# plainerman/DiffDock-Pocket

Measured on AMD Instinct MI355X. Metric: ligand poses/sec (40 samples x 20 steps) on 3dpf, higher is better.
Workload: dtype f32 (fc and G products: fp16 hi/lo split of both operands on v_mfma_f32_16x16x32_f16 - the row-stationary conv kernel - and v_mfma_f32_32x32x16_f16, fp32 accumulate; G between its two kernels as fp16 hi + continuation byte = 19 significant bits; the exact fp32 MFMA form is timed in other_workloads)

## Files before the change

### diffdock_pocket_amd/_lib.py

```python
from __future__ import annotations

import ctypes as C
import os

HERE = os.path.dirname(os.path.abspath(__file__))
LIB_PATH = os.environ.get("DDP_HIP_LIB", os.path.join(HERE, "libddp_hip.so"))

DDP_MAX_TASKS, DDP_MAX_BLOCKS, DDP_MAX_SEGS, DDP_MAX_NS, DDP_EDGE_TILE = 9, 4, 3, 64, 64
F_SCALAR_S0, F_DOT, F_SCALAR_S1, F_VEC_S0, F_CROSS = range(5)
FS = 68

DDP_MAX_GEMM_BATCH = 16
DDP_EVAL_MAX_ATOMS = 1024
EXPORTS = ["ddp_conv_messages", "ddp_conv_rows", "ddp_stage_a_gh", "ddp_stage_a_gh3", "ddp_segment_reduce", "ddp_edge_featurize", "ddp_edge_featurize_jobs", "ddp_torsion_sh", "ddp_stage_a", "ddp_stage_a_h2",
           "ddp_pose_update", "ddp_sidechain_update", "ddp_sde_update", "ddp_radius_count", "ddp_radius_fill", "ddp_knn", "ddp_group_by_key", "ddp_node_linear", "ddp_scan_jobs", "ddp_mark_jobs", "ddp_rowcopy_jobs", "ddp_select_jobs",
           "ddp_gather_rows", "ddp_clean_pair_maps", "ddp_flex_mark", "ddp_fallback_rowmap", "ddp_step_prologue", "ddp_trrot_head", "ddp_tor_head", "ddp_radius_search_jobs", "ddp_group_by_key_jobs", "ddp_set_occupancy_shaping", "ddp_pose_rmsd", "ddp_pose_contacts", "ddp_traj_record", "ddp_abi_version", "ddp_last_error", "ddp_source_hash"]


class Seg(C.Structure):
    _fields_ = [("kind", C.c_int32), ("in_off", C.c_int32), ("count", C.c_int32)]


class Block(C.Structure):
    _fields_ = [("U", C.c_int32), ("n", C.c_int32), ("C", C.c_int32), ("out_off", C.c_int32), ("tile0", C.c_int32),
                ("ntiles", C.c_int32), ("nsub", C.c_int32), ("ups", C.c_int32), ("nseg", C.c_int32),
                ("seg", Seg * DDP_MAX_SEGS), ("g_slot", C.c_int32), ("g_col0", C.c_int32)]


class RoleSeg(C.Structure):
    _fields_ = [("block", C.c_int32), ("tile0", C.c_int32), ("tstride", C.c_int32), ("count", C.c_int32), ("round", C.c_int32)]


DDP_CONV32_WAVES, DDP_MAX_ROLE_SEGS = 4, 2


class ConvShape(C.Structure):
    _fields_ = [("f_in", C.c_int32), ("hid", C.c_int32), ("kp1", C.c_int32), ("hp", C.c_int32), ("hs", C.c_int32),
                ("nct1", C.c_int32), ("d_out", C.c_int32), ("nblocks", C.c_int32), ("fbuf_floats", C.c_int32),
                ("g_cols", C.c_int32 * 2), ("blk", Block * DDP_MAX_BLOCKS), ("nrounds", C.c_int32),
                ("nrole", C.c_int32 * DDP_CONV32_WAVES), ("role", (RoleSeg * DDP_MAX_ROLE_SEGS) * DDP_CONV32_WAVES)]


class ConvTask(C.Structure):
    _fields_ = [("x_src", C.c_void_p), ("ldx_src", C.c_int32), ("n_edges", C.c_int32), ("src", C.c_void_p),
                ("eid", C.c_void_p), ("sh", C.c_void_p), ("seg_ptr", C.c_void_p * DDP_MAX_SEGS),
                ("seg_idx", C.c_void_p * DDP_MAX_SEGS), ("seg_ld", C.c_int32 * DDP_MAX_SEGS),
                ("seg_n", C.c_int32 * DDP_MAX_SEGS), ("w1p", C.c_void_p), ("b1p", C.c_void_p), ("w2p", C.c_void_p),
# ... 93 lines not shown


def g_ld(hid: int, gcols: int) -> int:
    return (((hid + 3) // 4 * 4 + 1) * gcols + 31) // 32 * 32


class DdpError(RuntimeError):
    pass


_lib = None


def load():
    global _lib
    if _lib is not None:
        return _lib
    if not os.path.exists(LIB_PATH):
        raise DdpError(f"{LIB_PATH} not found: build it with `python -m diffdock_pocket_amd.build` "
                       f"(hipcc --offload-arch=gfx950); there is no fallback path")
    lib = C.CDLL(LIB_PATH)
    for name in EXPORTS:
        if not hasattr(lib, name):
            raise DdpError(f"{LIB_PATH} does not export {name}")
    lib.ddp_abi_version.restype = C.c_int
    lib.ddp_last_error.restype = C.c_char_p
    lib.ddp_conv_messages.argtypes = [C.POINTER(ConvShape), C.POINTER(ConvTask), C.c_int, C.c_void_p]
    lib.ddp_conv_messages.restype = C.c_int
    lib.ddp_conv_rows.argtypes = lib.ddp_conv_messages.argtypes
    lib.ddp_conv_rows.restype = C.c_int
    lib.ddp_segment_reduce.argtypes = [C.c_void_p, C.c_int, C.c_int, C.c_int, C.POINTER(ReduceSrc), C.c_int, C.c_int,
                                       C.c_int, C.c_int, C.c_void_p]
    lib.ddp_segment_reduce.restype = C.c_int
    lib.ddp_edge_featurize.argtypes = [C.c_void_p, C.c_void_p, C.c_void_p, C.c_void_p, C.c_int, C.c_void_p, C.c_void_p, C.c_int,
                                       C.c_float, C.c_void_p, C.c_void_p, C.c_int, C.c_void_p, C.c_int, C.c_int, C.c_void_p,
                                       C.c_void_p, C.c_void_p, C.c_int, C.c_void_p, C.c_void_p, C.c_void_p]
    lib.ddp_edge_featurize.restype = C.c_int
    lib.ddp_edge_featurize_jobs.argtypes = [C.POINTER(FeaturizeJob), C.c_int, C.c_void_p]
    lib.ddp_edge_featurize_jobs.restype = C.c_int
    lib.ddp_torsion_sh.argtypes = [C.c_void_p, C.c_void_p, C.c_void_p, C.c_int, C.c_void_p, C.c_void_p, C.c_void_p, C.c_int, C.c_int,
                                   C.c_void_p, C.c_void_p, C.c_int, C.c_void_p, C.c_void_p]
    lib.ddp_torsion_sh.restype = C.c_int
    lib.ddp_stage_a.argtypes = [C.c_void_p, C.c_int, C.c_int, C.c_void_p, C.c_void_p, C.c_int, C.POINTER(C.c_int32), C.c_int,
                                C.c_void_p, C.c_void_p, C.c_int, C.c_int, C.c_void_p, C.c_int, C.c_void_p]
    lib.ddp_stage_a.restype = C.c_int
    lib.ddp_stage_a_h2.argtypes = lib.ddp_stage_a.argtypes[:-1] + [C.c_void_p, C.c_void_p]
    lib.ddp_stage_a_h2.restype = C.c_int
    lib.ddp_stage_a_gh.argtypes = lib.ddp_stage_a_h2.argtypes[:-1] + [C.c_void_p, C.c_void_p]
    lib.ddp_stage_a_gh.restype = C.c_int
    lib.ddp_stage_a_gh3.argtypes = lib.ddp_stage_a_gh.argtypes
    lib.ddp_stage_a_gh3.restype = C.c_int
    lib.ddp_set_occupancy_shaping.argtypes = [C.c_int, C.c_int]
    lib.ddp_set_occupancy_shaping.restype = C.c_int
    lib.ddp_pose_update.argtypes = [C.c_void_p, C.c_int, C.c_int, C.c_void_p, C.c_void_p, C.c_void_p, C.c_int, C.c_void_p,
                                    C.c_void_p, C.c_void_p, C.c_void_p]
    lib.ddp_pose_update.restype = C.c_int
    lib.ddp_sidechain_update.argtypes = [C.c_void_p, C.c_int, C.c_int, C.c_void_p, C.c_int, C.c_void_p, C.c_void_p, C.c_void_p,
                                         C.c_void_p, C.c_void_p]
    lib.ddp_sidechain_update.restype = C.c_int
    lib.ddp_radius_count.argtypes = [C.c_void_p, C.c_void_p, C.c_void_p, C.c_void_p, C.c_int, C.c_float, C.c_int, C.c_int,
                                     C.c_void_p, C.c_void_p]
    lib.ddp_radius_count.restype = C.c_int
    lib.ddp_radius_fill.argtypes = [C.c_void_p, C.c_void_p, C.c_void_p, C.c_void_p, C.c_int, C.c_float, C.c_int, C.c_int,
                                    C.c_void_p, C.c_void_p, C.c_void_p, C.c_void_p]
    lib.ddp_radius_fill.restype = C.c_int
    lib.ddp_knn.argtypes = [C.c_void_p, C.c_void_p, C.c_void_p, C.c_int, C.c_int, C.c_void_p, C.c_void_p]
# ... 50 lines not shown
```

### diffdock_pocket_amd/csrc/ddp_misc.hip

```cpp
#include <hip/hip_runtime.h>
#include <stdlib.h>
#include <stdint.h>

#include "ddp_hip.h"
#include "ddp_internal.h"

typedef float f32x4 __attribute__((ext_vector_type(4)));

struct ReduceLaunch {
  ddp_reduce_src_t src[3];
  int nsrc;
};

__global__ void ddp_segment_reduce_kernel(float* __restrict__ x, int ldx, int n_nodes, int d_out, ReduceLaunch L,
                                          int accumulate, int n_rep, int rep_stride) {
  const int node = blockIdx.x;
  const int ch = threadIdx.x;
  if (ch >= d_out) return;
  float* dst = x + (size_t)node * ldx + ch;
  float total = (accumulate && n_rep <= 1) ? *dst : 0.f;
  int p0[3], p1[3];
#pragma unroll
  for (int k = 0; k < 3; ++k) {
    const bool on = k < L.nsrc;
// ... 6 lines not shown
      const ddp_reduce_src_t& s = L.src[k];
      const float* __restrict__ m = s.msg + ch;
      const int32_t* __restrict__ rm = s.rowmap;
      float sum = 0.f;
      for (int p = p0[k]; p < p1[k]; p += 8) {
        float v[8];
        int row[8];
#pragma unroll
        for (int i = 0; i < 8; ++i) {
          const int q = min(p + i, p1[k] - 1);
          row[i] = rm ? rm[q] : q;
        }
#pragma unroll
        for (int i = 0; i < 8; ++i) v[i] = m[(size_t)row[i] * d_out];
#pragma unroll
        for (int i = 0; i < 8; ++i)
          if (p + i < p1[k]) sum += v[i];
      }
      const int cnt = p1[k] - p0[k];
      const float mean = sum / (float)(cnt > 1 ? cnt : 1);
      total += mean * s.bn_scale[ch] + s.bn_shift[ch];
    }
  }
  if (n_rep <= 1) {
    *dst = total;
  } else {
    for (int g = 0; g < n_rep; ++g) {
      float* d = dst + (size_t)g * rep_stride * ldx;
      *d = *d + total;
    }
  }
}

typedef float red4 __attribute__((ext_vector_type(4)));
__global__ __launch_bounds__(256) void ddp_segment_reduce4_kernel(float* __restrict__ x, int ldx, int n_nodes, int d_out, ReduceLaunch L,
                                                                  int accumulate, int n_rep, int rep_stride) {
  const int nq = d_out >> 2;
  const long long item = (long long)blockIdx.x * 256 + threadIdx.x;
  const int node = (int)(item / nq), ch = 4 * (int)(item - (long long)node * nq);
  if (node >= n_nodes) return;
  float* dst = x + (size_t)node * ldx + ch;
  red4 total = (accumulate && n_rep <= 1) ? *reinterpret_cast<const red4*>(dst) : red4{0.f, 0.f, 0.f, 0.f};
  int p0[3], p1[3];
#pragma unroll
  for (int k = 0; k < 3; ++k) {
    const bool on = k < L.nsrc;
    p0[k] = on ? L.src[k].rowptr[node] : 0;
    p1[k] = on ? L.src[k].rowptr[node + 1] : 0;
  }
#pragma unroll
  for (int k = 0; k < 3; ++k) {
    if (k < L.nsrc && !(L.src[k].n_edges_dev && *L.src[k].n_edges_dev <= 0)) {
      const ddp_reduce_src_t& s = L.src[k];
      const float* __restrict__ m = s.msg + ch;
      const int32_t* __restrict__ rm = s.rowmap;
      red4 sum = {0.f, 0.f, 0.f, 0.f};
      for (int p = p0[k]; p < p1[k]; p += 8) {
        red4 v[8];
        int row[8];
#pragma unroll
        for (int i = 0; i < 8; ++i) {
          const int q = min(p + i, p1[k] - 1);
          row[i] = rm ? rm[q] : q;
        }
#pragma unroll
        for (int i = 0; i < 8; ++i) v[i] = *reinterpret_cast<const red4*>(m + (size_t)row[i] * d_out);
#pragma unroll
        for (int i = 0; i < 8; ++i)
          if (p + i < p1[k]) sum += v[i];
      }
      const int cnt = p1[k] - p0[k];
      const float den = (float)(cnt > 1 ? cnt : 1);
      const red4 sc = *reinterpret_cast<const red4*>(s.bn_scale + ch), sh = *reinterpret_cast<const red4*>(s.bn_shift + ch);
#pragma unroll
      for (int c = 0; c < 4; ++c) total[c] += (sum[c] / den) * sc[c] + sh[c];
    }
  }
  if (n_rep <= 1) {
    *reinterpret_cast<red4*>(dst) = total;
  } else {
    for (int g = 0; g < n_rep; ++g) {
      red4* d = reinterpret_cast<red4*>(dst + (size_t)g * rep_stride * ldx);
      *d = *d + total;
    }
  }
}

extern "C" int ddp_segment_reduce(float* x, int ldx, int n_nodes, int d_out, const ddp_reduce_src_t* srcs, int nsrc,
                                  int accumulate, int n_rep, int rep_stride, void* stream) {
  if (!x || (!srcs && nsrc > 0)) return ddp_fail(DDP_EINVAL, "ddp_segment_reduce: null argument");
  if (nsrc < 0 || nsrc > 3) return ddp_fail(DDP_ELIMIT, "ddp_segment_reduce: nsrc > 3");
  if (d_out < 1 || d_out > 1024) return ddp_fail(DDP_ELIMIT, "ddp_segment_reduce: d_out");
  if (n_nodes <= 0) return 0;
  ReduceLaunch L;
  L.nsrc = 0;
  for (int i = 0; i < nsrc; ++i)
    if (srcs[i].n_edges > 0) L.src[L.nsrc++] = srcs[i];
  if (L.nsrc == 0 && (accumulate || n_rep > 1)) return 0;
  if (n_rep > 1 && rep_stride < n_nodes) return ddp_fail(DDP_EINVAL, "ddp_segment_reduce: rep_stride < n_nodes");
  bool wide = ((d_out | ldx) & 3) == 0 && (reinterpret_cast<size_t>(x) & 15) == 0;
  for (int i = 0; i < L.nsrc; ++i)
    wide = wide && ((reinterpret_cast<size_t>(L.src[i].msg) | reinterpret_cast<size_t>(L.src[i].bn_scale) | reinterpret_cast<size_t>(L.src[i].bn_shift)) & 15) == 0;
  static const bool narrow_only = getenv("DDP_REDUCE_NARROW") != nullptr;
  if (wide && !narrow_only) {
    const long long items = (long long)n_nodes * (d_out >> 2);
    hipLaunchKernelGGL(ddp_segment_reduce4_kernel, dim3((unsigned)((items + 255) / 256)), dim3(256), 0, (hipStream_t)stream, x, ldx, n_nodes,
                       d_out, L, accumulate, n_rep, rep_stride);
  } else {
    const int threads = ((d_out + 63) / 64) * 64;
    hipLaunchKernelGGL(ddp_segment_reduce_kernel, dim3(n_nodes), dim3(threads), 0, (hipStream_t)stream, x, ldx, n_nodes,
                       d_out, L, accumulate, n_rep, rep_stride);
  }
  hipError_t err = hipGetLastError();
  if (err != hipSuccess) return ddp_fail_hip(err, "ddp_segment_reduce launch");
  return 0;
}

#define EF_NS 64
__global__ __launch_bounds__(256) void ddp_edge_featurize_kernel(
    const float* __restrict__ pos_a, const int* __restrict__ ia, const float* __restrict__ pos_b,
    const int* __restrict__ ib, int n_edges, const int* __restrict__ n_edges_dev, const float* __restrict__ offset, int k_rbf,
    float coeff, const float* __restrict__ pre, const int* __restrict__ pre_idx, int ld_pre, const float* __restrict__ pre2,
    int n_pre2, int ld_pre2, const float* __restrict__ w1d, const float* __restrict__ w2, const float* __restrict__ b2, int ns,
    float* __restrict__ out, float* __restrict__ sh) {
  if (n_edges_dev) n_edges = min(n_edges, *n_edges_dev);
  extern __shared__ __attribute__((aligned(16))) float smem[];
  float* s_w1 = smem;
  float* s_w2 = s_w1 + k_rbf * EF_NS;
  float* s_b2 = s_w2 + EF_NS * EF_NS;
  float* s_off = s_b2 + EF_NS;
  float* s_out = s_off + ((k_rbf + 3) & ~3);
  const int tid = threadIdx.x;
  for (int i = tid; i < k_rbf * EF_NS; i += 256) s_w1[i] = w1d[i];
  for (int i = tid; i < EF_NS * EF_NS; i += 256) s_w2[i] = w2[i];
  if (tid < EF_NS) s_b2[tid] = b2[tid];
  for (int i = tid; i < k_rbf; i += 256) s_off[i] = offset[i];
  __syncthreads();

  const int wave = tid >> 6, lane = tid & 63;
  float* my_out = s_out + wave * 64 * 65;
  for (int base = blockIdx.x * 256; base < n_edges; base += gridDim.x * 256) {
    const int e = base + tid;
    const bool live = e < n_edges;
    const int ec = live ? e : n_edges - 1;
    const int a = ia[ec], b = ib[ec];
    const float vx = pos_b[3 * b] - pos_a[3 * a], vy = pos_b[3 * b + 1] - pos_a[3 * a + 1],
                vz = pos_b[3 * b + 2] - pos_a[3 * a + 2];
    const float d = sqrtf(vx * vx + vy * vy + vz * vz);
// ... 300 lines not shown
```

### diffdock_pocket_amd/engine.py

```python
from __future__ import annotations

import ctypes as C
from collections.abc import Mapping
from types import SimpleNamespace
from typing import Dict, List, Optional

import math

import torch

from . import _lib as L
from . import graph as G
from . import launch as K
from . import packing as P
from . import packing as P_
from .graph import EdgeView

SRC_TYPE = {0: "l", 1: "r", 2: "a", 3: "a", 4: "l", 5: "r", 6: "r", 7: "l", 8: "a"}
RECV_TYPE = {0: "l", 1: "l", 2: "l", 3: "a", 4: "a", 5: "a", 6: "r", 7: "r", 8: "r"}
RECV_OF = {"a": (3, 4, 5), "r": (6, 7, 8)}
ORDER = {"l": [0, 2, 1], "a": [3, 4, 5], "r": [6, 8, 7]}
_DROP_SELF = 1


# ... 798 lines not shown
                    if sd_.n_edges > 0:
                        segs = [(e_base, sd_.eid, ns, ns), (x_recv, sd_.recv, ldx, ns), (xa, sd_.src, ldx, ns)]
                        tasks_g.append(K.make_task(pkg, path, xa, ldx, sd_, sh_k, segs, msg, g=[P.g_d.get((3, s_)) for s_ in (0, 1)]))
                    sv = c1.so_v
                    segs = [(e_base, sv.eid, ns, ns), (P.x_clean, sv.recv, ldx, ns), (P.x_clean, sv.src, ldx, ns)]
                    tasks_g.append(K.make_task(pkg, path, P.x_clean, ldx, sv, sh_k, segs, msg, g=[P.g_v.get((3, s_)) for s_ in (0, 1)]))
                    continue
                msg = torch.empty((csr.n_edges, spec.d_out), device=dev)
                P.msgs[k] = (msg, csr, pkc)
                if csr.n_edges == 0:
                    continue
                if prof_on:
                    nb_g += node_bytes(l, k)
                segs = [(e_base, so_k.eid, ns, ns), (x_recv, so_k.recv, ldx, ns), (x_src, so_k.src, ldx, ns)]
                tasks_g.append(K.make_task(conv.packed_g(dev), self._conv_path(conv, dev), x_src, ldx, so_k, sh_k, segs, msg,
                                           g=[P.gmap.get((k, s_)) for s_ in (0, 1)]))
            P.tasks_g = getattr(P, "tasks_g", []) + tasks_g
            if tasks_g:
                K.launch_convs(P.spec_g, tasks_g, flops_spec=spec, node_bytes=nb_g, tag=f"layer{l}")

        def fix_rowmaps(P):
            if P.l == 0 and F.flex0 is not None:
                for k, rm in F.flex0.rowmaps.items():
                    if k in P.msgs:
                        P.msgs[k] = (P.msgs[k][0], c[k], P.msgs[k][2], rm)

        def means(P, types):
            spec, shared = P.spec, P.shared
            for rt in types:
                if not P.active[rt]:
                    continue
                x, n = nodes[rt]
                own = [P.msgs[k] for k in ORDER[rt] if k not in shared]
                if own:
                    K.launch_reduce(x, ldx, n, spec.d_out, own, accumulate=True)
                com = [P.msgs[k] for k in ORDER[rt] if k in shared]
                if com:
                    n0 = shared[[k for k in ORDER[rt] if k in shared][0]][0]
                    K.launch_reduce(x, ldx, n0, spec.d_out, com, accumulate=True, n_rep=B, rep_stride=n0)

        if pipelined:
            P = plan(0)
            direct_tasks(P)
            if P.tasks:
                side.run(1, lambda P=P: launch_direct(P))
            stage_a(P, "lar")
            def atom_g_bytes(Pn):
                tot = 0
                for (st_, _gid), (_x, rows_, convs_) in (Pn.groups.items() if m.rows_all_or_none(dev) else ()):
                    if st_ != "a":
                        continue
                    for _k, conv_ in convs_:
                        tot += rows_[3] * 4 * sum(ld_ for ld_ in (conv_.packed_g(dev).gh_ld or []) if ld_ is not None)
                return tot
            for l in range(L_):
                nxt = plan(l + 1) if l + 1 < L_ else None
                launch_factorised(P)
                join_lists()
                fix_rowmaps(P)
                side.join(only=1)
                side.join(only=0)
                ev_r, ev_l, ev_sr, ev_sl = (torch.cuda.Event() for _ in range(4))

                def rec_chain(P=P, nxt=nxt, ev_r=ev_r, ev_sr=ev_sr):
                    means(P, "r")
                    ev_r.record()
                    if nxt is not None:
                        stage_a(nxt, "r")
                        ev_sr.record()

                def lig_chain(P=P, nxt=nxt, ev_l=ev_l, ev_sl=ev_sl):
                    means(P, "l")
# ... 184 lines not shown
```

### diffdock_pocket_amd/launch.py

```python
from __future__ import annotations

import ctypes as C
import os
from dataclasses import dataclass
from typing import Dict, List, NamedTuple, Optional, Sequence

import torch
from torch import nn

from . import _lib as L
from . import packing as P
from .graph import EdgeView


def require_hip(t: torch.Tensor):
    if not t.is_cuda:
        raise L.DdpError("the MI355X score model runs on a HIP device only (no CPU/eager fallback); "
                         "move the batch to cuda:<n>")
    L.load()


def stream():
    return C.c_void_p(torch._C._cuda_getCurrentRawStream(torch._C._cuda_getDevice()))

# ... 204 lines not shown
    t.gh_fmt, t.rows_form, t.rows_bias_k, t.rows_nts = path.gh_fmt, path.rows_form, path.rows_bias_k, path.rows_nts
    t.rows_seg0, t.rows_seg1 = path.rows_seg
    t._path = path
    t.pos = _p(view.pos)
    t.n_edges_dev = _p(view.cnt)
    t._count = (view.n_edges, view.cnt)
    return t


def launch_convs(spec: P.ConvSpec, tasks: List[L.ConvTask], flops_spec: Optional[P.ConvSpec] = None, node_bytes: float = 0.0, tag=None):
    lib = L.load()
    if not tasks:
        return
    path = tasks[0]._path
    if any((t._path.rows, t._path.rows_form) != (path.rows, path.rows_form) for t in tasks):
        raise L.DdpError("launch_convs: the tasks of one launch run through different conv kernels")
    arr = (L.ConvTask * len(tasks))(*tasks)
    shape = spec.ctypes_shape()
    prof = _PROFILER
    if prof is not None:
        e0, e1 = torch.cuda.Event(enable_timing=True), torch.cuda.Event(enable_timing=True)
        e0.record()
    if path.rows:
        L.check(lib.ddp_conv_rows(C.byref(shape), arr, len(tasks), stream()), "ddp_conv_rows")
    else:
        L.check(lib.ddp_conv_messages(C.byref(shape), arr, len(tasks), stream()), "ddp_conv_messages")
    if prof is not None:
        e1.record()
        h2 = P.h2_steps(spec) > 0 and all(t._path.h2 for t in tasks)
        prof.record_conv(e0, e1, spec, flops_spec, [t._count for t in tasks], node_bytes, tag, h2,
                         rows=(2 if path.rows_form == 1 else 1) if path.rows else 0)


def launch_reduce(x, ldx, n_nodes, d_out, sources, accumulate=True, n_rep=1, rep_stride=0):
    lib = L.load()
    arr = (L.ReduceSrc * max(len(sources), 1))()
    for i, src_ in enumerate(sources):
        msg, view, pk = src_[:3]
        arr[i].msg, arr[i].rowptr = msg.data_ptr(), view.rowptr.data_ptr()
        arr[i].bn_scale, arr[i].bn_shift, arr[i].n_edges = pk.bn_scale.data_ptr(), pk.bn_shift.data_ptr(), view.n_edges
        arr[i].rowmap = src_[3].data_ptr() if (len(src_) > 3 and src_[3] is not None) else 0
        arr[i].n_edges_dev = _p(view.cnt)
    prof = profiler(hbm=True)
    if prof is not None:
        e0, e1 = torch.cuda.Event(enable_timing=True), torch.cuda.Event(enable_timing=True)
        e0.record()
    L.check(lib.ddp_segment_reduce(ptr(x), ldx, n_nodes, d_out, arr, len(sources), 1 if accumulate else 0, n_rep, rep_stride,
                                   stream()), "ddp_segment_reduce")
    if prof is not None:
        e1.record()
        views = [s_[1] for s_ in sources]

        def nbytes(views=views, d_out=d_out, n_nodes=n_nodes, n_rep=n_rep):
            ne = sum(v.n_edges if v.cnt is None else min(v.n_edges, int(v.cnt.item())) for v in views)
            return 4.0 * d_out * (ne + 2 * n_nodes * max(n_rep, 1))
        wide = (d_out % 4 == 0 and ldx % 4 == 0 and x.data_ptr() % 16 == 0 and not os.environ.get("DDP_REDUCE_NARROW")
                and all(s_[0].data_ptr() % 16 == 0 and s_[2].bn_scale.data_ptr() % 16 == 0 and s_[2].bn_shift.data_ptr() % 16 == 0 for s_ in sources))
        prof.hbm.setdefault("ddp_segment_reduce4_kernel" if wide else "ddp_segment_reduce_kernel", []).append((e0, e1, nbytes))


class EdgeMLPPack:

    def __init__(self, seq: nn.Sequential, rbf_slice: slice, device):
        W1, b1, W2, b2 = seq[0].weight.detach(), seq[0].bias.detach(), seq[3].weight.detach(), seq[3].bias.detach()
        ns = W1.shape[0]
        k = rbf_slice.stop - rbf_slice.start
        w1d = torch.zeros(k, 64, device=device)
        w1d[:, :ns] = W1[:, rbf_slice].t()
        w2 = torch.zeros(64, 64, device=device)
        w2[:ns, :ns] = W2.t()
        b2p = torch.zeros(64, device=device)
        b2p[:ns] = b2
        self.w1d, self.w2, self.b2, self.ns, self.k = w1d.contiguous(), w2.contiguous(), b2p, ns, k
        self.W1, self.b1 = W1, b1


def edge_featurize(pack: EdgeMLPPack, dist, pos_a, ia, pos_b, ib, pre, pre_idx, pre2=None, n_edges=None, cnt=None):
    lib = L.load()
    E = int(ia.shape[0]) if n_edges is None else int(n_edges)
    dev = pos_a.device
    out = torch.empty((E, pack.ns), device=dev, dtype=torch.float32)
    sh = torch.empty((E, 4), device=dev, dtype=torch.float32)
    if E == 0:
        return out, sh
    if pre.stride(1) != 1:
        pre = pre.contiguous()
    n2 = 0 if pre2 is None else int(pre2.shape[0])
    L.check(lib.ddp_edge_featurize(ptr(pos_a), ptr(ia), ptr(pos_b), ptr(ib), E, ptr(cnt), ptr(dist.offset), pack.k,
                                   C.c_float(dist.coeff), ptr(pre), ptr(pre_idx), pre.stride(0),
                                   ptr(pre2) if n2 else None, n2, pre2.stride(0) if n2 else 0, ptr(pack.w1d),
                                   ptr(pack.w2), ptr(pack.b2), pack.ns, ptr(out), ptr(sh), stream()),
# ... 248 lines not shown
```

### include/ddp_hip.h

```cpp
#ifndef DDP_HIP_H
#define DDP_HIP_H

#include <stdint.h>

#ifdef __cplusplus
extern "C" {
#endif

#define DDP_ABI_VERSION 17
#define DDP_EINVAL (-1)
#define DDP_ELIMIT (-2)

#define DDP_MAX_TASKS 9
#define DDP_MAX_BLOCKS 4
#define DDP_MAX_SEGS 3
#define DDP_MAX_NS 64
#define DDP_EDGE_TILE 64

enum ddp_feat_kind {
  DDP_F_SCALAR_S0 = 0,
  DDP_F_DOT = 1,
  DDP_F_SCALAR_S1 = 2,
  DDP_F_VEC_S0 = 3,
  DDP_F_CROSS = 4
// ... 66 lines not shown
  const void* w2h;
  int32_t* h2_range_flag;
  const void* wsh;
  const float* bsp;
  const void* gh[2];
  int32_t gh_fmt;
  int32_t rows_form;
  int32_t rows_bias_k;
  int32_t rows_seg0, rows_seg1, rows_nts;
} ddp_conv_task_t;
#define DDP_ROWS_SX 16
#define DDP_ROWS_SW 256
#define DDP_ROWS_SH 16
#define DDP_ROWS_SG 32
#define DDP_ROWS_KPERM(ks, hh, i) (32 * ((ks) >> 1) + ((8 * ((ks) & 1) + (i)) & 3) + 8 * ((8 * ((ks) & 1) + (i)) >> 2) + 4 * (hh))
#define DDP_ROWS16_POS(j) (16 * (((j) & 7) >> 2) + 4 * ((j) >> 3) + ((j) & 3))
#define DDP_GH3_LD(hid, gcp) ((((((hid) + 7) / 8) * (gcp) + ((gcp) + 5) / 6 + 15) / 16) * 96)
#define DDP_GH_LD(hid, gcp) ((((((hid) + 7) / 8) * 8 + 1) * (gcp) + 31) / 32 * 32)
int ddp_conv_messages(const ddp_conv_shape_t* shape, const ddp_conv_task_t* tasks, int ntasks, void* stream);

int ddp_conv_rows(const ddp_conv_shape_t* shape, const ddp_conv_task_t* tasks, int ntasks, void* stream);

typedef struct {
  const float* msg;
  const int32_t* rowptr;
  const float* bn_scale;
  const float* bn_shift;
  int32_t n_edges;
  const int32_t* rowmap;
  const int32_t* n_edges_dev;
} ddp_reduce_src_t;
int ddp_segment_reduce(float* x, int ldx, int n_nodes, int d_out, const ddp_reduce_src_t* srcs, int nsrc,
                       int accumulate, int n_rep, int rep_stride, void* stream);

int ddp_edge_featurize(const float* pos_a, const int32_t* ia, const float* pos_b, const int32_t* ib, int n_edges,
                       const int32_t* n_edges_dev, const float* offset, int k_rbf, float coeff, const float* pre,
                       const int32_t* pre_idx, int ld_pre, const float* pre2, int n_pre2, int ld_pre2, const float* w1d,
                       const float* w2, const float* b2, int ns, float* out, float* sh, void* stream);

#define DDP_MAX_FEATURIZE_JOBS 8
typedef struct {
  const float* pos_a;
  const int32_t* ia;
  const float* pos_b;
  const int32_t* ib;
  int32_t n_edges;
  const int32_t* n_edges_dev;
  const float* offset;
  int32_t k_rbf;
  float coeff;
  const float* pre;
  const int32_t* pre_idx;
  int32_t ld_pre;
  const float* pre2;
  int32_t n_pre2, ld_pre2;
  const float* w1d;
  const float* w2;
  const float* b2;
  int32_t ns;
  float* out;
  float* sh;
} ddp_featurize_job_t;
int ddp_edge_featurize_jobs(const ddp_featurize_job_t* jobs, int njobs, void* stream);

int ddp_torsion_sh(const float* sh_edge, const float* bond_vec, const int32_t* bond_of_edge, int n_edges,
                   const int32_t* n_edges_dev, float* out, const float* x, int ldx, int ns, const int32_t* b0,
// ... 255 lines not shown
```

Baseline: 173.3.

## Fuse own and shared segment reductions into one software-pipelined persistent kernel

```diff
diff --git a/diffdock_pocket_amd/_lib.py b/diffdock_pocket_amd/_lib.py
--- a/diffdock_pocket_amd/_lib.py
+++ b/diffdock_pocket_amd/_lib.py
@@ -12,7 +12,7 @@
 
 DDP_MAX_GEMM_BATCH = 16
 DDP_EVAL_MAX_ATOMS = 1024
-EXPORTS = ["ddp_conv_messages", "ddp_conv_rows", "ddp_stage_a_gh", "ddp_stage_a_gh3", "ddp_segment_reduce", "ddp_edge_featurize", "ddp_edge_featurize_jobs", "ddp_torsion_sh", "ddp_stage_a", "ddp_stage_a_h2",
+EXPORTS = ["ddp_conv_messages", "ddp_conv_rows", "ddp_stage_a_gh", "ddp_stage_a_gh3", "ddp_segment_reduce", "ddp_segment_reduce_fused", "ddp_edge_featurize", "ddp_edge_featurize_jobs", "ddp_torsion_sh", "ddp_stage_a", "ddp_stage_a_h2",
            "ddp_pose_update", "ddp_sidechain_update", "ddp_sde_update", "ddp_radius_count", "ddp_radius_fill", "ddp_knn", "ddp_group_by_key", "ddp_node_linear", "ddp_scan_jobs", "ddp_mark_jobs", "ddp_rowcopy_jobs", "ddp_select_jobs",
            "ddp_gather_rows", "ddp_clean_pair_maps", "ddp_flex_mark", "ddp_fallback_rowmap", "ddp_step_prologue", "ddp_trrot_head", "ddp_tor_head", "ddp_radius_search_jobs", "ddp_group_by_key_jobs", "ddp_set_occupancy_shaping", "ddp_pose_rmsd", "ddp_pose_contacts", "ddp_traj_record", "ddp_abi_version", "ddp_last_error", "ddp_source_hash"]
 
@@ -172,6 +172,9 @@
     lib.ddp_segment_reduce.argtypes = [C.c_void_p, C.c_int, C.c_int, C.c_int, C.POINTER(ReduceSrc), C.c_int, C.c_int,
                                        C.c_int, C.c_int, C.c_void_p]
     lib.ddp_segment_reduce.restype = C.c_int
+    lib.ddp_segment_reduce_fused.argtypes = [C.c_void_p, C.c_int, C.c_int, C.c_int, C.POINTER(ReduceSrc), C.c_int, C.POINTER(ReduceSrc), C.c_int,
+                                             C.c_int, C.c_int, C.c_int, C.c_void_p]
+    lib.ddp_segment_reduce_fused.restype = C.c_int
     lib.ddp_edge_featurize.argtypes = [C.c_void_p, C.c_void_p, C.c_void_p, C.c_void_p, C.c_int, C.c_void_p, C.c_void_p, C.c_int,
                                        C.c_float, C.c_void_p, C.c_void_p, C.c_int, C.c_void_p, C.c_int, C.c_int, C.c_void_p,
                                        C.c_void_p, C.c_void_p, C.c_int, C.c_void_p, C.c_void_p, C.c_void_p]
diff --git a/diffdock_pocket_amd/csrc/ddp_misc.hip b/diffdock_pocket_amd/csrc/ddp_misc.hip
--- a/diffdock_pocket_amd/csrc/ddp_misc.hip
+++ b/diffdock_pocket_amd/csrc/ddp_misc.hip
@@ -62,58 +62,265 @@
   }
 }
 
-typedef float red4 __attribute__((ext_vector_type(4)));
-__global__ __launch_bounds__(256) void ddp_segment_reduce4_kernel(float* __restrict__ x, int ldx, int n_nodes, int d_out, ReduceLaunch L,
-                                                                  int accumulate, int n_rep, int rep_stride) {
-  const int nq = d_out >> 2;
-  const long long item = (long long)blockIdx.x * 256 + threadIdx.x;
-  const int node = (int)(item / nq), ch = 4 * (int)(item - (long long)node * nq);
-  if (node >= n_nodes) return;
-  float* dst = x + (size_t)node * ldx + ch;
-  red4 total = (accumulate && n_rep <= 1) ? *reinterpret_cast<const red4*>(dst) : red4{0.f, 0.f, 0.f, 0.f};
+#define RP_ROWS 4
+struct PipeSrc {
+  const float* msg;
+  const int32_t* rowptr;
+  const float* bn_scale;
+  const float* bn_shift;
+  const int32_t* rowmap;
+  const int32_t* n_edges_dev;
+  int com;
+};
+struct PipeJob {
+  float* x;
+  int ldx, d_out;
+  int n_rows;
+  int n_own;
+  int accumulate;
+  int n0, n_rep, rep_stride;
+  int nsrc;
+  int lpn_log2, chunks;
+  PipeSrc src[3];
+};
+
+template <int V>
+__device__ __forceinline__ void rp_load(const float* p, float (&o)[V]) {
+  if constexpr (V == 1) {
+    o[0] = *p;
+  } else {
+    typedef float vec_t __attribute__((ext_vector_type(V)));
+    const vec_t t = *reinterpret_cast<const vec_t*>(p);
+#pragma unroll
+    for (int c = 0; c < V; ++c) o[c] = t[c];
+  }
+}
+template <int V>
+__device__ __forceinline__ void rp_store(float* p, const float (&o)[V]) {
+  if constexpr (V == 1) {
+    *p = o[0];
+  } else {
+    typedef float vec_t __attribute__((ext_vector_type(V)));
+    vec_t t;
+#pragma unroll
+    for (int c = 0; c < V; ++c) t[c] = o[c];
+    *reinterpret_cast<vec_t*>(p) = t;
+  }
+}
+
+struct PipePtrs {
   int p0[3], p1[3];
-#pragma unroll
-  for (int k = 0; k < 3; ++k) {
-    const bool on = k < L.nsrc;
-    p0[k] = on ? L.src[k].rowptr[node] : 0;
-    p1[k] = on ? L.src[k].rowptr[node + 1] : 0;
-  }
-#pragma unroll
-  for (int k = 0; k < 3; ++k) {
-    if (k < L.nsrc && !(L.src[k].n_edges_dev && *L.src[k].n_edges_dev <= 0)) {
-      const ddp_reduce_src_t& s = L.src[k];
-      const float* __restrict__ m = s.msg + ch;
-      const int32_t* __restrict__ rm = s.rowmap;
-      red4 sum = {0.f, 0.f, 0.f, 0.f};
-      for (int p = p0[k]; p < p1[k]; p += 8) {
-        red4 v[8];
-        int row[8];
-#pragma unroll
-        for (int i = 0; i < 8; ++i) {
-          const int q = min(p + i, p1[k] - 1);
-          row[i] = rm ? rm[q] : q;
+  int r, j, ch;
+};
+
+template <int V>
+__global__ __launch_bounds__(256) void ddp_segment_reduce_pipe_kernel(const PipeJob J) {
+  const int lpn = 1 << J.lpn_log2, lig = (int)threadIdx.x & (lpn - 1);
+  const int slot = (int)(((long long)blockIdx.x * 256 + threadIdx.x) >> J.lpn_log2);
+  const int nslots = (int)(((long long)gridDim.x * 256) >> J.lpn_log2);
+  const int n_items = J.n_rows * J.chunks;
+  const int d_out = J.d_out;
+  bool live[3];
+#pragma unroll
+  for (int k = 0; k < 3; ++k)
+    live[k] = k < J.nsrc && !(J.src[k].n_edges_dev && *J.src[k].n_edges_dev <= 0);
+
+  auto fetch_ptrs = [&](int it, PipePtrs& P) {
+#pragma unroll
+    for (int k = 0; k < 3; ++k) P.p0[k] = P.p1[k] = -1;
+    P.r = P.j = P.ch = -1;
+    if (it < n_items) {
+      const int r = it / J.chunks, chunk = it - r * J.chunks;
+      const int ch = ((chunk << J.lpn_log2) + lig) * V;
+      if (ch < d_out) {
+        P.r = r;
+        P.ch = ch;
+        if (J.n_rep >= 1) {
+          const int g = r / J.rep_stride, jj = r - g * J.rep_stride;
+          if (g < J.n_rep && jj < J.n0) P.j = jj;
         }
 #pragma unroll
-        for (int i = 0; i < 8; ++i) v[i] = *reinterpret_cast<const red4*>(m + (size_t)row[i] * d_out);
-#pragma unroll
-        for (int i = 0; i < 8; ++i)
-          if (p + i < p1[k]) sum += v[i];
-      }
-      const int cnt = p1[k] - p0[k];
-      const float den = (float)(cnt > 1 ? cnt : 1);
-      const red4 sc = *reinterpret_cast<const red4*>(s.bn_scale + ch), sh = *reinterpret_cast<const red4*>(s.bn_shift + ch);
-#pragma unroll
-      for (int c = 0; c < 4; ++c) total[c] += (sum[c] / den) * sc[c] + sh[c];
-    }
-  }
-  if (n_rep <= 1) {
-    *reinterpret_cast<red4*>(dst) = total;
-  } else {
-    for (int g = 0; g < n_rep; ++g) {
-      red4* d = reinterpret_cast<red4*>(dst + (size_t)g * rep_stride * ldx);
-      *d = *d + total;
-    }
-  }
+        for (int k = 0; k < 3; ++k)
+          if (live[k]) {
+            const int nk = J.src[k].com ? P.j : (r < J.n_own ? r : -1);
+            if (nk >= 0) {
+              P.p0[k] = J.src[k].rowptr[nk];
+              P.p1[k] = J.src[k].rowptr[nk + 1];
+            }
+          }
+      }
+    }
+  };
+  auto fetch_map = [&](const PipePtrs& P, int (&row)[3][RP_ROWS]) {
+#pragma unroll
+    for (int k = 0; k < 3; ++k) {
+      const int32_t* __restrict__ rm = k < J.nsrc ? J.src[k].rowmap : nullptr;
+#pragma unroll
+      for (int i = 0; i < RP_ROWS; ++i) {
+        const int q = P.p0[k] + i;
+        row[k][i] = (P.p0[k] >= 0 && q < P.p1[k]) ? (rm ? rm[q] : q) : -1;
+      }
+    }
+  };
+  auto fetch_rows = [&](const PipePtrs& P, const int (&row)[3][RP_ROWS], float (&v)[3][RP_ROWS][V], float (&xv)[V]) {
+#pragma unroll
+    for (int k = 0; k < 3; ++k)
+#pragma unroll
+      for (int i = 0; i < RP_ROWS; ++i)
+        if (row[k][i] >= 0) rp_load<V>(J.src[k].msg + (size_t)row[k][i] * d_out + P.ch, v[k][i]);
+    if (P.ch >= 0 && ((P.r < J.n_own && J.accumulate) || (P.r >= J.n_own && P.j >= 0)))
+      rp_load<V>(J.x + (size_t)P.r * J.ldx + P.ch, xv);
+  };
+  auto fetch_bn = [&](const PipePtrs& P, float (&sc)[3][V], float (&sh)[3][V]) {
+    if (P.ch < 0) return;
+#pragma unroll
+    for (int k = 0; k < 3; ++k)
+      if (k < J.nsrc) {
+        rp_load<V>(J.src[k].bn_scale + P.ch, sc[k]);
+        rp_load<V>(J.src[k].bn_shift + P.ch, sh[k]);
+      }
+  };
+
+  PipePtrs P, P1, P2;
+  int row[3][RP_ROWS];
+  float v[3][RP_ROWS][V], xv[V], sc[3][V], sh[3][V];
+#pragma unroll
+  for (int c = 0; c < V; ++c) xv[c] = 0.f;
+  fetch_ptrs(slot, P);
+  fetch_ptrs(slot + nslots, P1);
+  fetch_map(P, row);
+  fetch_rows(P, row, v, xv);
+  fetch_bn(P, sc, sh);
+  for (int it = slot; it < n_items; it += nslots) {
+    int row1[3][RP_ROWS];
+    fetch_map(P1, row1);
+    fetch_ptrs(it + 2 * nslots, P2);
+    if (P.ch >= 0) {
+      float total[V], ct[V];
+      const bool from_x = (P.r < J.n_own && J.accumulate) || (P.r >= J.n_own && P.j >= 0);
+#pragma unroll
+      for (int c = 0; c < V; ++c) {
+        total[c] = from_x ? xv[c] : 0.f;
+        ct[c] = 0.f;
+      }
+#pragma unroll
+      for (int k = 0; k < 3; ++k) {
+        if (P.p0[k] < 0) continue;
+        const PipeSrc& s = J.src[k];
+        float sum[V];
+#pragma unroll
+        for (int c = 0; c < V; ++c) sum[c] = 0.f;
+#pragma unroll
+        for (int i = 0; i < RP_ROWS; ++i)
+          if (P.p0[k] + i < P.p1[k]) {
+#pragma unroll
+            for (int c = 0; c < V; ++c) sum[c] += v[k][i][c];
+          }
+        const int32_t* __restrict__ rm = s.rowmap;
+        const float* __restrict__ m = s.msg + P.ch;
+        for (int p = P.p0[k] + RP_ROWS; p < P.p1[k]; p += RP_ROWS) {
+          int rw[RP_ROWS];
+          float t[RP_ROWS][V];
+#pragma unroll
+          for (int i = 0; i < RP_ROWS; ++i) rw[i] = p + i < P.p1[k] ? (rm ? rm[p + i] : p + i) : -1;
+#pragma unroll
+          for (int i = 0; i < RP_ROWS; ++i)
+            if (rw[i] >= 0) rp_load<V>(m + (size_t)rw[i] * d_out, t[i]);
+#pragma unroll
+          for (int i = 0; i < RP_ROWS; ++i)
+            if (rw[i] >= 0) {
+#pragma unroll
+              for (int c = 0; c < V; ++c) sum[c] += t[i][c];
+            }
+        }
+        const int cnt = P.p1[k] - P.p0[k];
+        const float den = (float)(cnt > 1 ? cnt : 1);
+        if (s.com == 1) {
+#pragma unroll
+          for (int c = 0; c < V; ++c) ct[c] += (sum[c] / den) * sc[k][c] + sh[k][c];
+        } else {
+#pragma unroll
+          for (int c = 0; c < V; ++c) total[c] += (sum[c] / den) * sc[k][c] + sh[k][c];
+        }
+      }
+      if (P.j >= 0 && J.n_rep > 1) {
+#pragma unroll
+        for (int c = 0; c < V; ++c) total[c] = total[c] + ct[c];
+      }
+      if (P.r < J.n_own || P.j >= 0) rp_store<V>(J.x + (size_t)P.r * J.ldx + P.ch, total);
+    }
+    P = P1;
+    P1 = P2;
+#pragma unroll
+    for (int k = 0; k < 3; ++k)
+#pragma unroll
+      for (int i = 0; i < RP_ROWS; ++i) row[k][i] = row1[k][i];
+    fetch_rows(P, row, v, xv);
+    if (J.chunks > 1) fetch_bn(P, sc, sh);
+  }
+}
+
+template <int V>
+static long long reduce_grid_cap() {
+  static long long cap = 0;
+  if (cap == 0) {
+    int dev = 0, cus = 0, per_cu = 0;
+    if (hipGetDevice(&dev) != hipSuccess || hipDeviceGetAttribute(&cus, hipDeviceAttributeMultiprocessorCount, dev) != hipSuccess || cus <= 0) cus = 256;
+    if (hipOccupancyMaxActiveBlocksPerMultiprocessor(&per_cu, ddp_segment_reduce_pipe_kernel<V>, 256, 0) != hipSuccess || per_cu < 1) per_cu = 2;
+    (void)hipGetLastError();
+    cap = (long long)cus * (per_cu < 4 ? per_cu : 4);
+  }
+  return cap;
+}
+
+static int reduce_launch(const char* who, float* x, int ldx, int d_out, int n_own, const ddp_reduce_src_t* own, int n_own_src, int accumulate,
+                         const ddp_reduce_src_t* com, int n_com_src, int n0, int n_rep, int rep_stride, void* stream) {
+  PipeJob J;
+  J.x = x; J.ldx = ldx; J.d_out = d_out; J.n_own = n_own; J.accumulate = accumulate;
+  J.nsrc = 0;
+  for (int i = 0; i < n_own_src; ++i)
+    if (own[i].n_edges > 0 && n_own > 0) {
+      const ddp_reduce_src_t& s = own[i];
+      J.src[J.nsrc++] = PipeSrc{s.msg, s.rowptr, s.bn_scale, s.bn_shift, s.rowmap, s.n_edges_dev, 0};
+    }
+  const int n_own_live = J.nsrc;
+  for (int i = 0; i < n_com_src; ++i)
+    if (com[i].n_edges > 0 && n0 > 0 && n_rep >= 1) {
+      const ddp_reduce_src_t& s = com[i];
+      J.src[J.nsrc++] = PipeSrc{s.msg, s.rowptr, s.bn_scale, s.bn_shift, s.rowmap, s.n_edges_dev, n_rep > 1 ? 1 : 2};
+    }
+  const bool has_com = J.nsrc > n_own_live;
+  if (n_own_live == 0 && accumulate) J.n_own = 0;
+  J.n0 = has_com ? n0 : 0;
+  J.n_rep = has_com ? n_rep : 0;
+  J.rep_stride = has_com ? (n_rep > 1 ? rep_stride : n0) : 1;
+  long long rows = J.n_own;
+  if (has_com && (long long)(J.n_rep - 1) * J.rep_stride + J.n0 > rows) rows = (long long)(J.n_rep - 1) * J.rep_stride + J.n0;
+  if (rows <= 0) return 0;
+  for (int k = J.nsrc; k < 3; ++k) J.src[k] = PipeSrc{nullptr, nullptr, nullptr, nullptr, nullptr, nullptr, 0};
+  for (int k = 0; k < J.nsrc; ++k)
+    if (!J.src[k].msg || !J.src[k].rowptr || !J.src[k].bn_scale || !J.src[k].bn_shift) return ddp_fail(DDP_EINVAL, "segment reduce: a source with a null array");
+  size_t al = reinterpret_cast<size_t>(x) | ((size_t)ldx * 4) | ((size_t)d_out * 4);
+  for (int k = 0; k < J.nsrc; ++k)
+    al |= reinterpret_cast<size_t>(J.src[k].msg) | reinterpret_cast<size_t>(J.src[k].bn_scale) | reinterpret_cast<size_t>(J.src[k].bn_shift);
+  const int V = (al & 15) == 0 ? 4 : (al & 7) == 0 ? 2 : 1;
+  const int nvec = d_out / V;
+  int lg = 0;
+  while ((1 << lg) < nvec && lg < 6) ++lg;
+  J.lpn_log2 = lg;
+  J.chunks = (nvec + (1 << lg) - 1) >> lg;
+  if (rows * J.chunks > 0x7fe00000LL) return ddp_fail(DDP_ELIMIT, who);
+  J.n_rows = (int)rows;
+  const long long lanes = (rows * J.chunks) << lg;
+  long long blocks = (lanes + 255) / 256;
+  const long long cap = V == 4 ? reduce_grid_cap<4>() : V == 2 ? reduce_grid_cap<2>() : reduce_grid_cap<1>();
+  if (blocks > cap) blocks = cap;
+  if (V == 4) hipLaunchKernelGGL(ddp_segment_reduce_pipe_kernel<4>, dim3((unsigned)blocks), dim3(256), 0, (hipStream_t)stream, J);
+  else if (V == 2) hipLaunchKernelGGL(ddp_segment_reduce_pipe_kernel<2>, dim3((unsigned)blocks), dim3(256), 0, (hipStream_t)stream, J);
+  else hipLaunchKernelGGL(ddp_segment_reduce_pipe_kernel<1>, dim3((unsigned)blocks), dim3(256), 0, (hipStream_t)stream, J);
+  hipError_t err = hipGetLastError();
+  if (err != hipSuccess) return ddp_fail_hip(err, who);
+  return 0;
 }
 
 extern "C" int ddp_segment_reduce(float* x, int ldx, int n_nodes, int d_out, const ddp_reduce_src_t* srcs, int nsrc,
@@ -128,22 +335,31 @@
     if (srcs[i].n_edges > 0) L.src[L.nsrc++] = srcs[i];
   if (L.nsrc == 0 && (accumulate || n_rep > 1)) return 0;
   if (n_rep > 1 && rep_stride < n_nodes) return ddp_fail(DDP_EINVAL, "ddp_segment_reduce: rep_stride < n_nodes");
-  bool wide = ((d_out | ldx) & 3) == 0 && (reinterpret_cast<size_t>(x) & 15) == 0;
-  for (int i = 0; i < L.nsrc; ++i)
-    wide = wide && ((reinterpret_cast<size_t>(L.src[i].msg) | reinterpret_cast<size_t>(L.src[i].bn_scale) | reinterpret_cast<size_t>(L.src[i].bn_shift)) & 15) == 0;
-  static const bool narrow_only = getenv("DDP_REDUCE_NARROW") != nullptr;
-  if (wide && !narrow_only) {
-    const long long items = (long long)n_nodes * (d_out >> 2);
-    hipLaunchKernelGGL(ddp_segment_reduce4_kernel, dim3((unsigned)((items + 255) / 256)), dim3(256), 0, (hipStream_t)stream, x, ldx, n_nodes,
-                       d_out, L, accumulate, n_rep, rep_stride);
-  } else {
+  if (getenv("DDP_REDUCE_NARROW") != nullptr) {
     const int threads = ((d_out + 63) / 64) * 64;
     hipLaunchKernelGGL(ddp_segment_reduce_kernel, dim3(n_nodes), dim3(threads), 0, (hipStream_t)stream, x, ldx, n_nodes,
                        d_out, L, accumulate, n_rep, rep_stride);
-  }
-  hipError_t err = hipGetLastError();
-  if (err != hipSuccess) return ddp_fail_hip(err, "ddp_segment_reduce launch");
-  return 0;
+    hipError_t err = hipGetLastError();
+    if (err != hipSuccess) return ddp_fail_hip(err, "ddp_segment_reduce launch");
+    return 0;
+  }
+  if (n_rep > 1) return reduce_launch("ddp_segment_reduce launch", x, ldx, d_out, 0, nullptr, 0, 1, L.src, L.nsrc, n_nodes, n_rep, rep_stride, stream);
+  return reduce_launch("ddp_segment_reduce launch", x, ldx, d_out, n_nodes, L.src, L.nsrc, accumulate, nullptr, 0, 0, 0, 0, stream);
+}
+
+extern "C" int ddp_segment_reduce_fused(float* x, int ldx, int n_nodes, int d_out, const ddp_reduce_src_t* own, int n_own_src,
+                                        const ddp_reduce_src_t* com, int n_com_src, int n0, int n_rep, int rep_stride, void* stream) {
+  if (!x || (!own && n_own_src > 0) || (!com && n_com_src > 0)) return ddp_fail(DDP_EINVAL, "ddp_segment_reduce_fused: null argument");
+  if (n_own_src < 0 || n_com_src < 0 || n_own_src > 3 || n_com_src > 3 || n_own_src + n_com_src > 3)
+    return ddp_fail(DDP_ELIMIT, "ddp_segment_reduce_fused: more than 3 sources");
+  if (d_out < 1 || d_out > 1024) return ddp_fail(DDP_ELIMIT, "ddp_segment_reduce_fused: d_out");
+  if (ldx < d_out) return ddp_fail(DDP_EINVAL, "ddp_segment_reduce_fused: ldx < d_out");
+  if (n_com_src > 0 && n0 > 0) {
+    if (n_rep < 1) return ddp_fail(DDP_EINVAL, "ddp_segment_reduce_fused: n_rep < 1");
+    if (n_rep > 1 && rep_stride < n0) return ddp_fail(DDP_EINVAL, "ddp_segment_reduce_fused: rep_stride < n0");
+  }
+  if (n_nodes < 0) n_nodes = 0;
+  return reduce_launch("ddp_segment_reduce_fused launch", x, ldx, d_out, n_nodes, own, n_own_src, 1, com, n_com_src, n0, n_rep, rep_stride, stream);
 }
 
 #define EF_NS 64
diff --git a/diffdock_pocket_amd/engine.py b/diffdock_pocket_amd/engine.py
--- a/diffdock_pocket_amd/engine.py
+++ b/diffdock_pocket_amd/engine.py
@@ -854,12 +854,12 @@
                     continue
                 x, n = nodes[rt]
                 own = [P.msgs[k] for k in ORDER[rt] if k not in shared]
-                if own:
-                    K.launch_reduce(x, ldx, n, spec.d_out, own, accumulate=True)
                 com = [P.msgs[k] for k in ORDER[rt] if k in shared]
                 if com:
                     n0 = shared[[k for k in ORDER[rt] if k in shared][0]][0]
-                    K.launch_reduce(x, ldx, n0, spec.d_out, com, accumulate=True, n_rep=B, rep_stride=n0)
+                    K.launch_reduce_fused(x, ldx, n, spec.d_out, own, com, n0, B, n0)
+                elif own:
+                    K.launch_reduce(x, ldx, n, spec.d_out, own, accumulate=True)
 
         if pipelined:
             P = plan(0)
diff --git a/diffdock_pocket_amd/launch.py b/diffdock_pocket_amd/launch.py
--- a/diffdock_pocket_amd/launch.py
+++ b/diffdock_pocket_amd/launch.py
@@ -260,8 +260,7 @@
                          rows=(2 if path.rows_form == 1 else 1) if path.rows else 0)
 
 
-def launch_reduce(x, ldx, n_nodes, d_out, sources, accumulate=True, n_rep=1, rep_stride=0):
-    lib = L.load()
+def _reduce_sources(sources):
     arr = (L.ReduceSrc * max(len(sources), 1))()
     for i, src_ in enumerate(sources):
         msg, view, pk = src_[:3]
@@ -269,6 +268,22 @@
         arr[i].bn_scale, arr[i].bn_shift, arr[i].n_edges = pk.bn_scale.data_ptr(), pk.bn_shift.data_ptr(), view.n_edges
         arr[i].rowmap = src_[3].data_ptr() if (len(src_) > 3 and src_[3] is not None) else 0
         arr[i].n_edges_dev = _p(view.cnt)
+    return arr
+
+
+def _reduce_key(x, ldx, d_out, sources):
+    wide = (d_out % 2 == 0 and ldx % 2 == 0 and x.data_ptr() % 8 == 0 and "DDP_REDUCE_NARROW" not in os.environ
+            and all(s_[0].data_ptr() % 8 == 0 and s_[2].bn_scale.data_ptr() % 8 == 0 and s_[2].bn_shift.data_ptr() % 8 == 0 for s_ in sources))
+    return "ddp_segment_reduce4_kernel" if wide else "ddp_segment_reduce_kernel"
+
+
+def _reduce_edges(views):
+    return sum(v.n_edges if v.cnt is None else min(v.n_edges, int(v.cnt.item())) for v in views)
+
+
+def launch_reduce(x, ldx, n_nodes, d_out, sources, accumulate=True, n_rep=1, rep_stride=0):
+    lib = L.load()
+    arr = _reduce_sources(sources)
     prof = profiler(hbm=True)
     if prof is not None:
         e0, e1 = torch.cuda.Event(enable_timing=True), torch.cuda.Event(enable_timing=True)
@@ -280,11 +295,26 @@
         views = [s_[1] for s_ in sources]
 
         def nbytes(views=views, d_out=d_out, n_nodes=n_nodes, n_rep=n_rep):
-            ne = sum(v.n_edges if v.cnt is None else min(v.n_edges, int(v.cnt.item())) for v in views)
-            return 4.0 * d_out * (ne + 2 * n_nodes * max(n_rep, 1))
-        wide = (d_out % 4 == 0 and ldx % 4 == 0 and x.data_ptr() % 16 == 0 and not os.environ.get("DDP_REDUCE_NARROW")
-                and all(s_[0].data_ptr() % 16 == 0 and s_[2].bn_scale.data_ptr() % 16 == 0 and s_[2].bn_shift.data_ptr() % 16 == 0 for s_ in sources))
-        prof.hbm.setdefault("ddp_segment_reduce4_kernel" if wide else "ddp_segment_reduce_kernel", []).append((e0, e1, nbytes))
+            return 4.0 * d_out * (_reduce_edges(views) + 2 * n_nodes * max(n_rep, 1))
+        prof.hbm.setdefault(_reduce_key(x, ldx, d_out, sources), []).append((e0, e1, nbytes))
+
+
+def launch_reduce_fused(x, ldx, n_nodes, d_out, own, com, n0, n_rep, rep_stride):
+    lib = L.load()
+    a_own, a_com = _reduce_sources(own), _reduce_sources(com)
+    prof = profiler(hbm=True)
+    if prof is not None:
+        e0, e1 = torch.cuda.Event(enable_timing=True), torch.cuda.Event(enable_timing=True)
+        e0.record()
+    L.check(lib.ddp_segment_reduce_fused(ptr(x), ldx, n_nodes, d_out, a_own, len(own), a_com, len(com), n0, n_rep, rep_stride, stream()),
+            "ddp_segment_reduce_fused")
+    if prof is not None:
+        e1.record()
+        v_own, v_com = [s_[1] for s_ in own], [s_[1] for s_ in com]
+
+        def nbytes(v_own=v_own, v_com=v_com, d_out=d_out, n_nodes=n_nodes):
+            return 4.0 * d_out * (_reduce_edges(v_own) + _reduce_edges(v_com) + 2 * n_nodes)
+        prof.hbm.setdefault(_reduce_key(x, ldx, d_out, list(own) + list(com)), []).append((e0, e1, nbytes))
 
 
 class EdgeMLPPack:
diff --git a/include/ddp_hip.h b/include/ddp_hip.h
--- a/include/ddp_hip.h
+++ b/include/ddp_hip.h
@@ -122,6 +122,8 @@
 } ddp_reduce_src_t;
 int ddp_segment_reduce(float* x, int ldx, int n_nodes, int d_out, const ddp_reduce_src_t* srcs, int nsrc,
                        int accumulate, int n_rep, int rep_stride, void* stream);
+int ddp_segment_reduce_fused(float* x, int ldx, int n_nodes, int d_out, const ddp_reduce_src_t* own, int n_own_src,
+                             const ddp_reduce_src_t* com, int n_com_src, int n0, int n_rep, int rep_stride, void* stream);
 
 int ddp_edge_featurize(const float* pos_a, const int32_t* ia, const float* pos_b, const int32_t* ib, int n_edges,
                        const int32_t* n_edges_dev, const float* offset, int k_rbf, float coeff, const float* pre,
```

Result: slower. 171.6 (-1.0%).
